# wondmgezahu/RAMP

Measured on AMD Instinct MI355X. Metric: sampled trajectories/sec (H=48, T=25), higher is better.
Workload: dtype f32-emulated (2 x fp16 planes per operand, fp32 accumulate)

## Files before the change

ramp_amd/csrc/args_token.h:

```cpp
#pragma once
#include "core.h"

namespace ramp {

struct FfxArgs {
  int M = 0;
  const float* X = nullptr;
  const float* Z1 = nullptr;
  float* Y = nullptr;
  float* stash = nullptr;
  const float* ln_g = nullptr; const float* ln_b = nullptr;
  const unsigned short* Wstream = nullptr;
  const float* b1 = nullptr;
  const float* b2 = nullptr;
  const float* amax_in1 = nullptr; float* amax_out1 = nullptr; float wsi1 = 1.f; int site1 = 0;
  const float* amax_in2 = nullptr; float* amax_out2 = nullptr; float wsi2 = 1.f; int site2 = 0;
  int* range_flag = nullptr;
  unsigned long long* stamps = nullptr;
  int ablate = 0;
  int tok0 = 0, slot0 = 0, half_mode = 0;
};
int launch_ffx(const FfxArgs& f, bool bwd, hipStream_t s);
int ffx_pack_second(const float* W, int rows, int cols, int mode, float scale, float* tmp, unsigned short* out, hipStream_t s);
int ffx_build_stream(const unsigned short* p1, const unsigned short* p2, unsigned short* out, bool bwd, hipStream_t s);
int init_ffx_attributes();
int launch_ffx16(const FfxArgs& f, bool bwd, hipStream_t s);
int ffx16_pack(const float* W, int rows, int cols, int perm, float scale, float* tmp, unsigned short* out, hipStream_t s);
int ffx16_build_stream(const unsigned short* p1, const unsigned short* p2, unsigned short* out, bool bwd, hipStream_t s);
int init_ffx16_attributes();

struct TklArgs {
  int M = 0, N = 0;
  const float* X = nullptr;
  float* Y = nullptr; int ldy = 0;
  const unsigned short* W = nullptr;
  const float* bias = nullptr;
  const float* resid = nullptr; int ldr = 0;
  const float* rowbias = nullptr; const int* rowvar = nullptr; int row0 = 0, rb_stride = 0, L = 1, n_var = 0;
  const float* ln_g = nullptr; const float* ln_b = nullptr;
  const float* amax_in = nullptr; float* amax_out = nullptr; float wsi = 1.f; int site = 0;
  int* range_flag = nullptr;
  int ablate = 0;
};
// ... 18 lines not shown
```

ramp_amd/csrc/engine.hip:

```cpp
#include "engine_util.h"

#include <algorithm>
#include <array>
#include <cmath>
#include <cstring>
#include <map>
#include <memory>
#include <mutex>
#include <string>
#include <unordered_map>
#include <vector>

namespace ramp {

static thread_local std::string g_err;
void set_last_error(const std::string& msg) { g_err = msg; }
int device_cu_count() {
  static int cached[64] = {0};
  int dev = 0;
  if (hipGetDevice(&dev) != hipSuccess || dev < 0 || dev >= 64) return 256;
  if (!cached[dev]) {
    hipDeviceProp_t p;
    cached[dev] = hipGetDeviceProperties(&p, dev) == hipSuccess && p.multiProcessorCount > 0 ? p.multiProcessorCount : 256;
  }
// ... 22 lines not shown
  float *w1_f = nullptr, *w1_b = nullptr, *b1 = nullptr, *w2_f = nullptr, *w2_b = nullptr, *b2 = nullptr;
  float *w1_pk = nullptr, *b1_pk = nullptr;
  float *ln1_g = nullptr, *ln1_b = nullptr, *ln3_g = nullptr, *ln3_b = nullptr;
  const float *wv2 = nullptr, *wo2 = nullptr, *bo2 = nullptr;
  float *a_qkv = nullptr, *a_z1 = nullptr, *a_ag = nullptr, *a_z2 = nullptr;
  unsigned short *ffx_f = nullptr, *ffx_b = nullptr; float ffx_wsi_w1 = 1.f, ffx_wsi_w2 = 1.f;
  unsigned short *ffx16_f = nullptr, *ffx16_b = nullptr;
  unsigned short* ato_w = nullptr; float ato_wsi = 1.f;
  unsigned short* abl_w = nullptr;
};
struct ST {
  std::string name;
  int C = 0, L = 0, blk0 = 0;
  float *gn_g = nullptr, *gn_b = nullptr, *wpi_f = nullptr, *wpi_b = nullptr, *bpi = nullptr;
  float *wpo_f = nullptr, *wpo_b = nullptr, *bpo = nullptr;
  STBlock blk[2];
  float *a_gst = nullptr, *a_z0 = nullptr, *a_y = nullptr;
};
struct Resample {
  std::string name;
  float *w_f = nullptr, *w_b = nullptr, *bias = nullptr;
  int C = 0, Lin = 0, Lout = 0, taps = 0;
  float* a_y = nullptr;
};

}

using namespace ramp;

#ifndef RAMP_DEFAULT_GEMM_MODE
// ... 32 lines not shown
  bool c_cal_valid = false; std::string c_cal_key; unsigned long long* c_cal_rec = nullptr;
  std::map<std::string, float*> c_cal_saved;
  std::vector<float*> c_cal_free;
  float *r_noise = nullptr, *r_hist = nullptr, *r_xclean = nullptr, *r_best = nullptr, *r_plen = nullptr, *r_smooth = nullptr,
        *r_cost = nullptr, *r_hard_val = nullptr;
  double *r_static = nullptr, *r_dyn = nullptr;
  int *r_mask = nullptr, *r_en = nullptr, *r_result = nullptr, *r_hard_idx = nullptr;
  ReplanState* r_state = nullptr;
  size_t r_cap_B = 0, r_cap_static = 0, r_cap_dyn = 0, r_cap_cost = 0;
  hipGraphExec_t r_graph[2] = {nullptr, nullptr}; std::string r_key;
  bool r_calibrated = false;
  float* scene_ws = nullptr; size_t scene_ws_cap = 0;
  int gemm_mode = 0;
  struct X6W { unsigned short* planes; size_t n; int K; unsigned short* packed; unsigned short* packed3; float w_scale_inv; };
  std::map<const float*, X6W> x6;
  int x6_pipe = 1;
  int geglu_group = 64;
  static constexpr int MAX_SITES = 1024, N_OBS_TABLES = 4;
  int phase = 0, site = 0;
  int ff_fused = 150000;
  int three_blocks = 1;
  int mfma16 = 1;
  int ffx_min_rows = 32768;
  int tkl_min_rows = 65536;
  int atk_min_rows = 40000;
  int tkc_gn = 3;
  int tkc_min_rows = 16384;
  int tkw_min_rows = 16384;
  std::map<const float*, unsigned short*> tk16_w;
  struct TkcW { unsigned short* planes; float wsi; };
// ... 146 lines not shown
    CK(get_raw(c, t + ".norm1.weight", {D}, &k.ln1_g)); CK(get_raw(c, t + ".norm1.bias", {D}, &k.ln1_b));
    CK(get_raw(c, t + ".norm3.weight", {D}, &k.ln3_g)); CK(get_raw(c, t + ".norm3.bias", {D}, &k.ln3_b));
    float* tmp;
    CK(get_raw(c, t + ".attn2.to_v.weight", {D, ctx}, &tmp)); k.wv2 = tmp;
    CK(get_raw(c, t + ".attn2.to_out.0.weight", {D, D}, &tmp)); k.wo2 = tmp;
    CK(get_raw(c, t + ".attn2.to_out.0.bias", {D}, &tmp)); k.bo2 = tmp;
    CK(get_raw(c, t + ".attn2.to_q.weight", {D, D}, &tmp));
    CK(get_raw(c, t + ".attn2.to_k.weight", {D, ctx}, &tmp));
    CK(get_raw(c, t + ".norm2.weight", {D}, &tmp)); CK(get_raw(c, t + ".norm2.bias", {D}, &tmp));
    CK(dev_alloc(c, &k.a_qkv, tok * 768)); CK(dev_alloc(c, &k.a_z1, tok * D));
    CK(dev_alloc(c, &k.a_ag, (tok + 127) * 2048)); CK(dev_alloc(c, &k.a_z2, tok * D));
  }
  return 0;
}

struct Run {
  ramp_ctx* c; hipStream_t s; int R; int row0;
  int prep(GemmArgs& b) {
    if (!(c->gemm_mode >= 1 && (b.N >= 128 || (c->x6_pipe && b.N >= 64)))) return 0;
    auto it = c->x6.upper_bound(b.W);
    if (it == c->x6.begin()) return 0;
    --it;
    const auto& e = it->second;
    if (!(b.W >= it->first && b.W < it->first + e.n)) return 0;
    const size_t off = b.W - it->first;
    const bool frag = c->x6_pipe && e.packed && e.K == b.K && off % (32ul * b.K) == 0 && b.N % 32 == 0;
    if (!frag) { b.Wx = e.planes + off; b.wx_plane = (long)e.n; return 0; }
    RAMP_REQUIRE(c->site < ramp_ctx::MAX_SITES, "too many GEMM call sites for the scale table");
    int kind = 1;
    if (c->phase == 2 && e.packed3) {
// ... 64 lines not shown
  int gemm(const GemmArgs& a) {
    if (const ramp_ctx::TkcW* w = tkc_planes(a)) return tkc(a, *w);
    prof_pre(c, s, CAT_GEMM, 2.0 * a.M * a.N * a.K * a.taps, {a.M, a.N, a.K, a.taps});
    GemmArgs b = a;
    b.three_ok = c->three_blocks;
    const int kind = prep(b);
    if (kind < 0) return kind;
    int rc = launch_gemm(b, s);
    prof_post(c, s);
    c->launches++;
    return rc;
  }
  bool use_ffx(const STBlock& k, int M) const {
    return k.ffx_f && c->ffx_min_rows > 0 && M >= c->ffx_min_rows && c->gemm_mode == 2 && c->phase == 2 && c->x6_pipe;
  }
  int ffx(const STBlock& k, bool bwd, const float* X, const float* z1, float* Y, int M) {
    RAMP_REQUIRE(c->site + 2 <= ramp_ctx::MAX_SITES, "too many GEMM call sites for the scale table");
    prof_pre(c, s, CAT_GEMM, 2.0 * M * (2048.0 * 256 + 256.0 * 1024), {M, bwd ? -3 : -2, 256, 2});
    FfxArgs f; f.M = M; f.X = X; f.Z1 = z1; f.Y = Y; f.stash = k.a_ag; f.ln_g = k.ln3_g; f.ln_b = k.ln3_b;
    const bool s16 = c->mfma16 && k.ffx16_f;
    f.Wstream = s16 ? (bwd ? k.ffx16_b : k.ffx16_f) : (bwd ? k.ffx_b : k.ffx_f); f.b1 = k.b1_pk; f.b2 = k.b2; f.range_flag = c->range_flag;
    f.amax_in1 = c->obs_in + c->site; f.amax_out1 = c->obs_out + c->site; f.site1 = c->site;
    f.amax_in2 = c->obs_in + c->site + 1; f.amax_out2 = c->obs_out + c->site + 1; f.site2 = c->site + 1;
    f.wsi1 = bwd ? k.ffx_wsi_w2 : k.ffx_wsi_w1; f.wsi2 = bwd ? k.ffx_wsi_w1 : k.ffx_wsi_w2;
    f.ablate = s16 ? 0 : c->ffx_ablate;
    c->site += 2;
    int rc = s16 ? launch_ffx16(f, bwd, s) : launch_ffx(f, bwd, s);
    prof_post(c, s);
    c->launches++;
    return rc;
  }
  bool has_h3(const float* W, int N, int K) const {
    auto it = c->x6.upper_bound(W);
    if (it == c->x6.begin()) return false;
    --it;
    const auto& e = it->second;
    if (!(W >= it->first && W < it->first + e.n)) return false;
    const size_t off = W - it->first;
    return c->x6_pipe && e.packed && e.packed3 && e.K == K && off % (32ul * K) == 0 && N % 32 == 0;
  }
  bool use_tkl(const GemmArgs& a) const {
// ... 237 lines not shown
        LAUNCH(c, r.s, CAT_ROW, 0, launch_ln_fwd(zin, k.ln1_g, k.ln1_b, c->t_ln, Mb, r.s));
        CK(r.gemm(q));
      }
    }
    const float* rowbias = c->cross_bias + (size_t)(m.blk0 + b) * D; const int rb_stride = c->n_blocks_total * D;
    if (r.use_ato(k, Mb, m.L)) {
      CK(r.ato(k, k.a_qkv, zin, pre ? c->t_ln : k.a_z1, Mb, m.L, pre ? nullptr : rowbias, rb_stride));
    } else {
    LAUNCH(c, r.s, CAT_ATTN, 16.0 * Rb * m.L * m.L * 64, launch_attn_fwd(k.a_qkv, c->t_o, Rb, m.L, r.s));
    GemmArgs a = lin(c->t_o, D, k.wo_f, k.bo, pre ? c->t_ln : k.a_z1, D, Mb, D, D);
    a.resid = zin; a.ldr = D; a.L = m.L;
    if (!pre) { a.rowbias = rowbias; a.rb_stride = rb_stride; a.rowvar = c->row_variant; a.row0 = r.row0; }
    if (r.use_tkl(a) && (!a.rowbias || c->n_variants <= 4)) CK(r.tkl(a, nullptr, nullptr)); else CK(r.gemm(a));
    }
    if (pre) LAUNCH(c, r.s, CAT_ROW, 0, launch_expand_rows(c->t_ln, k.a_z1, R, share, m.L, D, rowbias, rb_stride, c->row_variant, r.row0, r.s));
    if (r.use_ffx(k, M)) {
      CK(r.ffx(k, false, k.a_z1, k.a_z1, k.a_z2, M));
      zin = k.a_z2;
      continue;
    }
    LAUNCH(c, r.s, CAT_ROW, 0, launch_ln_fwd(k.a_z1, k.ln3_g, k.ln3_b, c->t_ln, M, r.s));
    GemmArgs u = lin(c->t_ln, D, k.w1_pk, k.b1_pk, k.a_ag, 2048, M, 2048, D);
    u.epi = EPI_GEGLU_FWD; u.aux_out = c->t_hg; u.ld_aux = 1024;
    u.geglu_group = c->geglu_group;
    GemmArgs f = lin(c->t_hg, 1024, k.w2_f, k.b2, k.a_z2, D, M, D, 1024);
    f.resid = k.a_z1; f.ldr = D;
    CK(r.ff_forward(u, f));
    zin = k.a_z2;
  }
  GemmArgs o = lin(zin, D, m.wpo_f, m.bpo, m.a_y, m.C, M, m.C, D);
// ... 388 lines not shown
    if (const char* me = getenv("RAMP_MFMA16")) c->mfma16 = atoi(me) != 0;
    const char* ke = getenv("RAMP_TKL");
    if (ke) c->tkl_min_rows = atoi(ke);
    const char* tce = getenv("RAMP_TKC");
    if (tce) c->tkc_min_rows = atoi(tce);
    if (const char* tg = getenv("RAMP_TKC_GN")) c->tkc_gn = atoi(tg) & 3;
    const char* twe = getenv("RAMP_TKW");
    if (twe) c->tkw_min_rows = atoi(twe);
    const char* ate = getenv("RAMP_ATK");
    if (ate) c->atk_min_rows = atoi(ate);
    const char* se = getenv("RAMP_SHARE_PREFIX");
    if (se) c->share_prefix = atoi(se) != 0;
    const char* te = getenv("RAMP_X6_THREE");
    if (te) c->three_blocks = te[0] != '0';
    c->prof_dump = getenv("RAMP_PROFILE_DUMP") != nullptr;
    const char* ae = getenv("RAMP_FFX_ABLATE");
    if (ae) {
      const int av = atoi(ae);
      if (!(av == 0 || av == 16 || av == 32 || av == 48)) {
        delete c;
        RAMP_REQUIRE(false, "RAMP_FFX_ABLATE accepts 0, 16, 32 or 48 (result-preserving variants) on a context; the others change results and exist in ramp_bench_gemm only");
      }
      c->ffx_ablate = av;
    }
    c->tklb_off = getenv("RAMP_TKLB_OFF") != nullptr;
    if (const char* e = getenv("RAMP_ABL")) c->abl_on = atoi(e) != 0;
  }
  *out = c;
  return 0;
}
// ... 194 lines not shown
          const auto& e1 = c->x6.at(k.w1_pk); const auto& e1b = c->x6.at(k.w1_b);
          const auto& e2 = c->x6.at(k.w2_f); const auto& e2b = c->x6.at(k.w2_b);
          RAMP_REQUIRE(e1.packed3 && e2b.packed3 && e1.w_scale_inv == e1b.w_scale_inv && e2.w_scale_inv == e2b.w_scale_inv, "ffx: weight planes missing");
          float *sf, *sb; CK(dev_alloc(c, &sf, 96 * 8192 + 4)); CK(dev_alloc(c, &sb, 96 * 8192 + 4));
          k.ffx_f = reinterpret_cast<unsigned short*>(sf); k.ffx_b = reinterpret_cast<unsigned short*>(sb);
          CK(ffx_pack_second(k.w2_f, 256, 1024, 0, 1.f / e2.w_scale_inv, tmp, p2f, 0));
          CK(ffx_build_stream(e1.packed3, p2f, k.ffx_f, false, 0));
          CK(ffx_pack_second(k.w1_b, 256, 2048, 1, 1.f / e1.w_scale_inv, tmp, p2b, 0));
          CK(ffx_build_stream(e2b.packed3, p2b, k.ffx_b, true, 0));
          k.ffx_wsi_w1 = e1.w_scale_inv; k.ffx_wsi_w2 = e2.w_scale_inv;
          float *sf6, *sb6; CK(dev_alloc(c, &sf6, 96 * 8192 + 4)); CK(dev_alloc(c, &sb6, 96 * 8192 + 4));
          k.ffx16_f = reinterpret_cast<unsigned short*>(sf6); k.ffx16_b = reinterpret_cast<unsigned short*>(sb6);
          CK(ffx16_pack(k.w1_pk, 2048, 256, 0, 1.f / e1.w_scale_inv, tmp, p1x, 0));
          CK(ffx16_pack(k.w2_f, 256, 1024, 1, 1.f / e2.w_scale_inv, tmp, p2f, 0));
          CK(ffx16_build_stream(p1x, p2f, k.ffx16_f, false, 0));
          CK(ffx16_pack(k.w2_b, 1024, 256, 0, 1.f / e2.w_scale_inv, tmp, p1x, 0));
          CK(ffx16_pack(k.w1_b, 256, 2048, 2, 1.f / e1.w_scale_inv, tmp, p2b, 0));
          CK(ffx16_build_stream(p1x, p2b, k.ffx16_b, true, 0));
          for (const auto& wn : {std::make_pair((const float*)k.wqkv_f, 768), std::make_pair((const float*)k.wo_f, 256), std::make_pair((const float*)k.wo_b, 256)}) {
            const auto& ew = c->x6.at(wn.first);
            if (!ew.packed3) continue;
            float* q16; CK(dev_alloc(c, &q16, (size_t)wn.second * 256 + 4));
            CK(ffx16_pack(wn.first, wn.second, 256, 0, 1.f / ew.w_scale_inv, tmp, reinterpret_cast<unsigned short*>(q16), 0));
            c->tk16_w[wn.first] = reinterpret_cast<unsigned short*>(q16);
          }
        }
    }
    if (c->gemm_mode == 2 && c->x6_pipe) {
      for (auto& st : c->sts)
        for (auto& k : st.blk) {
// ... 730 lines not shown
```

ramp_amd/csrc/ffx16.hip:

```cpp
#include "args_token.h"
#include "pack.h"
#include "tokmma.h"
#include "atkmma.h"

#include <algorithm>
#include <type_traits>

namespace ramp {

namespace {

constexpr int F6_SLAB = 32 * 1024;
constexpr int F6_R = 4;
constexpr int F6_B1 = F6_R * F6_SLAB;
constexpr int F6_LN = F6_B1 + 2048 * 4;
constexpr int F6_B2 = F6_LN + 512 * 4;
constexpr size_t F6_LDS = (size_t)F6_R * F6_SLAB + 2048 * 4 + 512 * 4 + 256 * 4;
constexpr int F6_SLABS = 96;
static_assert(F6_LDS <= 160 * 1024, "LDS budget");

enum { Q_P1A = 0, Q_P1B = 1, Q_P2A = 2, Q_P2B = 3 };
template <int V> using QO = std::integral_constant<int, V>;

}

namespace {
__device__ __forceinline__ void split2x(float x0, float x1, float s, unsigned& hi, unsigned& lo) {
  unsigned h, l;
  asm("v_fma_mixlo_f16 %0, %1, %3, 0 op_sel:[0,0,0] op_sel_hi:[0,0,0]\n\t"
      "v_fma_mixhi_f16 %0, %2, %3, 0 op_sel:[0,0,0] op_sel_hi:[0,0,0]"
      : "=&v"(h) : "v"(x0), "v"(x1), "v"(s));
  asm("v_fma_mixlo_f16 %0, %1, %3, -%4 op_sel:[0,0,0] op_sel_hi:[0,0,1]\n\t"
      "v_fma_mixhi_f16 %0, %2, %3, -%4 op_sel:[0,0,1] op_sel_hi:[0,0,1]"
      : "=&v"(l) : "v"(x0), "v"(x1), "v"(s), "v"(h));
  hi = h; lo = l;
}
}

template <bool BWD, int ABL, int NT>
__device__ __forceinline__ void ffx16_body(const FfxArgs& f, int n_mt) {
  static_assert(NT == 1 || NT == 2, "token halves");
  constexpr int NQ = 2 * NT;
  extern __shared__ __attribute__((aligned(16))) char smem[];
  const int tid = threadIdx.x, lane = tid & 63;
  const int wave = __builtin_amdgcn_readfirstlane(tid >> 6);
  const int c = lane & 15, gq = lane >> 4;
  const int n_my = (n_mt - (int)blockIdx.x + (int)gridDim.x - 1) / (int)gridDim.x;

  const float s_1 = scale_of(f.amax_in1), s_2 = scale_of(f.amax_in2);
  const float os1 = f.wsi1 / s_1, os2 = f.wsi2 / s_2;
  float amax1 = 0.f, amax2 = 0.f;
  const unsigned long long t_start = (ABL & 64) ? __builtin_amdgcn_s_memtime() : 0, r_start = (ABL & 64) ? __builtin_amdgcn_s_memrealtime() : 0;

  const char* wsrc = reinterpret_cast<const char*>(f.Wstream) + wave * 8192 + lane * 16;
  int is_q = 0, is_g = 0;
  const char* cur_src = wsrc; unsigned cur_dst = 0;
  auto dma_begin = [&]() __attribute__((always_inline)) {
    cur_src = wsrc + (long)is_q * F6_SLAB;
    cur_dst = (unsigned)(uintptr_t)(smem + (is_g & (F6_R - 1)) * F6_SLAB + wave * 8192);
    is_q = is_q + 1 == F6_SLABS ? 0 : is_q + 1;
    ++is_g;
  };
#define F6_PIECE(C) asm volatile("s_mov_b32 m0, %1\n\ts_nop 0\n\tglobal_load_lds_dwordx4 %0, off offset:%2" \
                                 :: "v"(cur_src + ((C) >> 2) * 4096), "s"(cur_dst + ((C) >> 2) * 4096), "n"(((C) & 3) * 1024) : "memory", "m0")
  auto dma_piece = [&](int cc) __attribute__((always_inline)) {
    switch (cc) { case 0: F6_PIECE(0); break; case 1: F6_PIECE(1); break; case 2: F6_PIECE(2); break; case 3: F6_PIECE(3); break;
                  case 4: F6_PIECE(4); break; case 5: F6_PIECE(5); break; case 6: F6_PIECE(6); break; default: F6_PIECE(7); break; }
  };
  auto issue_slab = [&]() __attribute__((always_inline)) {
    dma_begin();
#pragma unroll
    for (int cc = 0; cc < 8; ++cc) dma_piece(cc);
  };

  u32x4 F[3][4];
// ... 18 lines not shown
  f32x4 st1[BWD ? NQ : 1], st2[BWD ? NQ : 1];
  const f32x4 zero4 = {0.f, 0.f, 0.f, 0.f};

#define F6_MM(ACC, FA, BB, Z) ACC = mm32(FA, BB, (Z) ? zero4 : ACC)

  auto slab = [&](auto kind_c, auto fo_c, int par, auto side, auto vm_c) __attribute__((always_inline)) {
    constexpr int KIND = decltype(kind_c)::value, FO = decltype(fo_c)::value;
    slab_top(vm_c);
    const int slot = g & (F6_R - 1), nslot = (g + 1) & (F6_R - 1);
#pragma unroll
    for (int m = 0; m < 8; ++m) {
      u32x4 (&FB)[4] = F[(m + FO) % 3];
      u32x4 (&FN)[4] = F[(m + 2 + FO) % 3];
      const char* np = rd + (m < 6 ? slot * F6_SLAB + (m + 2) * 4096 : nslot * F6_SLAB + (m - 6) * 4096);
      constexpr bool P1 = KIND == Q_P1A || KIND == Q_P1B;
      const bool Z = P1 && m == 0;
      constexpr int T1 = NT - 1;
      f32x4* X0; f32x4* X1; f32x4* Y0; f32x4* Y1;
      const u32x4 (*BP)[2]; const u32x4 (*BQ)[2];
      if constexpr (!BWD) {
        if constexpr (P1) {
          X0 = &acc1[par][0][KIND]; X1 = &acc1[par][0][2 * T1 + KIND]; Y0 = &acc1[par][1][KIND]; Y1 = &acc1[par][1][2 * T1 + KIND];
          BP = XB[m]; BQ = XB[m];
        } else {
          X0 = &acc2[2 * m][0]; X1 = &acc2[2 * m][T1]; Y0 = &acc2[2 * m + 1][0]; Y1 = &acc2[2 * m + 1][T1];
          BP = HB; BQ = HB;
        }
      } else {
        if constexpr (P1) {
          X0 = &acc1[par][0][0]; X1 = &acc1[par][0][2 * T1]; Y0 = &acc1[par][0][1]; Y1 = &acc1[par][0][2 * T1 + 1];
          BP = XB[m]; BQ = XB[m];
        } else {
          const int nt = 8 * (KIND - Q_P2A) + m;
          X0 = &acc2[nt][0]; X1 = &acc2[nt][T1]; Y0 = X0; Y1 = X1;
          BP = HB; BQ = HB + NT;
// ... 290 lines not shown
      slab(KD{}, QO<0>{}, 0, [&](int m) __attribute__((always_inline)) { E_step(31, 1, 8 + m, 20, 16); }, V8{});
#pragma unroll
      for (int i = 16; i < 20; ++i) E_step(31, 1, i, 20, 16);
      slab(KC{}, QO<2>{}, 0, no_side, V8{}); slab(KD{}, QO<1>{}, 0, no_side, V8{});
    }
    asm volatile("s_nop 15\n\ts_nop 15" ::: "memory");

    int mt_e = mt;
    asm volatile("" : "+s"(mt_e));
    long tok_e[NT];
#pragma unroll
    for (int t = 0; t < NT; ++t) {
      tok_e[t] = (NT == 2 ? (long)mt_e * 128 + wave * 32 : (long)f.tok0 + (long)mt_e * 64 + wave * 16) + 16 * t + c;
      tok_e[t] = tok_e[t] < f.M ? tok_e[t] : f.M - 1;
    }
    if (!BWD) {
      const float* b2s = reinterpret_cast<const float*>(smem + F6_B2) + 4 * gq;
      f32x4 rz[NT][16];
#pragma unroll
      for (int t = 0; t < NT; ++t) {
        const float* zrow = f.Z1 + tok_e[t] * 256 + 4 * gq;
#pragma unroll
        for (int nt = 0; nt < 16; ++nt) rz[t][nt] = *reinterpret_cast<const f32x4*>(zrow + 16 * nt);
      }
#pragma unroll
      for (int t = 0; t < NT; ++t) {
        float* orow = f.Y + tok_e[t] * 256 + 4 * gq;
#pragma unroll
        for (int nt = 0; nt < 16; ++nt) {
          const f32x4 b2 = *reinterpret_cast<const f32x4*>(b2s + 16 * nt);
          const f32x4 v = acc2[nt][t] * os2 + b2 + rz[t][nt];
// ... 52 lines not shown
#undef F6_PIECE
#undef F6_MM
  if ((ABL & 64) && f.stamps && lane == 0) {
    unsigned long long* o = f.stamps + ((long)blockIdx.x * 4 + wave) * 6;
    o[0] = 0; o[1] = 0; o[2] = 0; o[3] = 0;
    o[4] = __builtin_amdgcn_s_memtime() - t_start;
    o[5] = __builtin_amdgcn_s_memrealtime() - r_start;
  }

  asm volatile("s_waitcnt vmcnt(0)" ::: "memory");

#pragma unroll
  for (int o = 32; o > 0; o >>= 1) { amax1 = fmaxf(amax1, __shfl_xor(amax1, o)); amax2 = fmaxf(amax2, __shfl_xor(amax2, o)); }
  record_amax_block(f.amax_out1, amax1, reinterpret_cast<float*>(smem));
  record_amax_block(f.amax_out2, amax2, reinterpret_cast<float*>(smem) + 4);
  if (lane == 0) {
    if (f.range_flag) {
      if (!(amax1 * s_1 < 60000.f) || (amax1 > 0.f && amax1 * s_1 < 0.125f)) atomicMax(f.range_flag, f.site1 + 1);
      if (!(amax2 * s_2 < 60000.f) || (amax2 > 0.f && amax2 * s_2 < 0.125f)) atomicMax(f.range_flag, f.site2 + 1);
    }
  }
}

template <bool BWD, int ABL = 0>
__global__ __launch_bounds__(256) __attribute__((amdgpu_waves_per_eu(1, 1)))
void ffx16_kernel(FfxArgs f, int n_mt) { ffx16_body<BWD, ABL, 2>(f, n_mt); }
template <bool BWD>
__global__ __launch_bounds__(256) __attribute__((amdgpu_waves_per_eu(1, 1)))
void ffx16h_kernel(FfxArgs f, int n_mt) { ffx16_body<BWD, 0, 1>(f, n_mt); }

__global__ void ffx16_gather_kernel(const float* __restrict__ in, float* __restrict__ out, int rows, int cols, int perm) {
  const long total = (long)rows * cols;
  const int oc = cols / 2;
  for (long idx = (long)blockIdx.x * 256 + threadIdx.x; idx < total; idx += (long)gridDim.x * 256) {
    const long orow = idx / oc; const int ocol = (int)(idx - orow * oc);
    const long R = orow >> 5; const int b = (int)(orow >> 4) & 1, cc = (int)orow & 15;
    const int s = ocol >> 4, h = (ocol >> 3) & 1, j = ocol & 7;
    const long srow = 16 * R + cc;
    const int pcol = 32 * s + 16 * h + 8 * b + j;
    const int gq = (pcol >> 3) & 3, jj = pcol & 7;
    int scol = pcol;
    if (perm == 1) scol = (pcol & ~31) + 16 * (jj >> 2) + 4 * gq + (jj & 3);
    else if (perm == 2) { const int u = pcol >> 6, w = (pcol >> 5) & 1; scol = (w ? 1024 : 0) + 32 * u + 16 * (jj >> 2) + 4 * gq + (jj & 3); }
    out[idx] = in[srow * cols + scol];
  }
}
int ffx16_pack(const float* W, int rows, int cols, int perm, float scale, float* tmp, unsigned short* out, hipStream_t s) {
  RAMP_REQUIRE(W && tmp && out && rows % 16 == 0 && cols % 32 == 0 && perm >= 0 && perm <= 2 && (perm != 2 || cols == 2048), "ffx16_pack: bad shape");
  hipLaunchKernelGGL(ffx16_gather_kernel, dim3(1024), dim3(256), 0, s, W, tmp, rows, cols, perm);
  RAMP_HIP_CHECK(hipGetLastError());
  return launch_pack_h3(tmp, out, 2L * rows, cols / 2, scale, s);
}

__global__ void ffx16_build_stream_kernel(const unsigned short* __restrict__ p1, const unsigned short* __restrict__ p2,
                                          unsigned short* __restrict__ out, int bwd) {
  const int q = blockIdx.x;
  int kind, u;
  if (!bwd) {
    if (q < 4) { kind = q & 1; u = q >> 1; }
    else if (q < 94) { const int k = 1 + (q - 4) / 3, j = (q - 4) - 3 * (k - 1); if (j == 0) { kind = Q_P2A; u = k - 1; } else { kind = j - 1; u = k + 1; } }
    else { kind = Q_P2A; u = q - 64; }
  } else {
    if (q < 2) { kind = Q_P1A; u = q; }
    else if (q < 92) { const int k = 1 + (q - 2) / 3, j = (q - 2) - 3 * (k - 1); if (j == 2) { kind = Q_P1A; u = k + 1; } else { kind = Q_P2A + j; u = k - 1; } }
    else { kind = Q_P2A + (q & 1); u = 30 + ((q - 92) >> 1); }
  }
  for (int i = threadIdx.x >> 6; i < 32; i += blockDim.x >> 6) {
    const int m = i >> 2, j = i & 3, lane = threadIdx.x & 63;
    const int pq = j >> 1, plane = j & 1;
    long frag;
    const unsigned short* base;
    if (!bwd) {
      if (kind <= Q_P1B) { base = p1; frag = (long)(4 * u + 2 * pq + kind) * 8 + m; }
      else { base = p2; frag = (long)(2 * m + pq) * 32 + u; }
    } else {
      if (kind == Q_P1A) { base = p1; frag = (long)(2 * u + pq) * 8 + m; }
      else { base = p2; frag = (long)(8 * (kind - Q_P2A) + m) * 64 + 2 * u + pq; }
    }
    reinterpret_cast<u32x4*>(out + ((long)q * 32 + i) * 512)[lane] = reinterpret_cast<const u32x4*>(base + (frag * 2 + plane) * 512)[lane];
  }
}
int ffx16_build_stream(const unsigned short* p1, const unsigned short* p2, unsigned short* out, bool bwd, hipStream_t s) {
  RAMP_REQUIRE(p1 && p2 && out, "ffx16_build_stream: null operand");
  hipLaunchKernelGGL(ffx16_build_stream_kernel, dim3(F6_SLABS), dim3(256), 0, s, p1, p2, out, bwd ? 1 : 0);
  RAMP_HIP_CHECK(hipGetLastError());
  return 0;
}

int launch_ffx16(const FfxArgs& f, bool bwd, hipStream_t s) {
  auto al16 = [](const void* p) { return (reinterpret_cast<uintptr_t>(p) & 15) == 0; };
  RAMP_REQUIRE(f.M > 0 && f.X && f.Y && f.Z1 && f.stash && f.Wstream && f.ln_g && (bwd || (f.ln_b && f.b1 && f.b2)), "ffx16: null operand");
  RAMP_REQUIRE(al16(f.X) && al16(f.Y) && al16(f.Z1) && al16(f.stash) && al16(f.Wstream) && al16(f.ln_g) && al16(f.ln_b) &&
               al16(f.b1) && al16(f.b2), "ffx16: operands must be 16-byte aligned");
  {
    const size_t yb = (size_t)f.M * 256 * 4;
    RAMP_REQUIRE(!ranges_overlap(f.Y, yb, f.X, yb) && !ranges_overlap(f.Y, yb, f.Z1, yb), "ffx16: the output must not overlap X or z1 (no in-place use)");
  }
  const int n_mt = (f.M + 127) / 128, cus = device_cu_count();
  RAMP_REQUIRE(f.half_mode >= 0 && f.half_mode <= 2 && (f.half_mode == 0 || f.ablate == 0), "ffx16: bad tiling mode");
  int n_full = n_mt;
  if (f.half_mode == 2) n_full = 0;
  else if (f.half_mode == 0 && f.ablate == 0) {
    const int r = n_mt % cus;
    if (2 * n_mt <= cus) n_full = 0;
    else if (n_mt > cus && r > 0 && 2 * r <= cus) n_full = n_mt - r;
  }
#define F6_GO(B, A) hipLaunchKernelGGL((ffx16_kernel<B, A>), dim3(std::min(n_full, cus)), dim3(256), F6_LDS, s, f, n_full)
  if (n_full > 0) {
    if (f.ablate == 0) { if (bwd) F6_GO(true, 0); else F6_GO(false, 0); }
    else if (f.ablate == 1) { if (bwd) F6_GO(true, 1); else F6_GO(false, 1); }
    else if (f.ablate == 64) { if (bwd) F6_GO(true, 64); else F6_GO(false, 64); }
    else RAMP_REQUIRE(false, "ffx16: ablation variant not built");
    RAMP_HIP_CHECK(hipGetLastError());
  }
#undef F6_GO
  if (n_full < n_mt) {
    FfxArgs h = f;
    h.tok0 = n_full * 128; h.slot0 = n_full;
    const int n_half = (f.M - h.tok0 + 63) / 64;
    if (bwd) hipLaunchKernelGGL((ffx16h_kernel<true>), dim3(std::min(n_half, cus)), dim3(256), F6_LDS, s, h, n_half);
    else hipLaunchKernelGGL((ffx16h_kernel<false>), dim3(std::min(n_half, cus)), dim3(256), F6_LDS, s, h, n_half);
    RAMP_HIP_CHECK(hipGetLastError());
  }
  return 0;
}

int init_ffx16_attributes() {
#define F6_ATTR(B, A) RAMP_HIP_CHECK(hipFuncSetAttribute(reinterpret_cast<const void*>(&ffx16_kernel<B, A>), hipFuncAttributeMaxDynamicSharedMemorySize, (int)F6_LDS))
  F6_ATTR(false, 0); F6_ATTR(true, 0); F6_ATTR(false, 1); F6_ATTR(true, 1); F6_ATTR(false, 64); F6_ATTR(true, 64);
#undef F6_ATTR
  RAMP_HIP_CHECK(hipFuncSetAttribute(reinterpret_cast<const void*>(&ffx16h_kernel<false>), hipFuncAttributeMaxDynamicSharedMemorySize, (int)F6_LDS));
  RAMP_HIP_CHECK(hipFuncSetAttribute(reinterpret_cast<const void*>(&ffx16h_kernel<true>), hipFuncAttributeMaxDynamicSharedMemorySize, (int)F6_LDS));
  return 0;
}

}
```

Before: 3962.

## Fuse spatial-transformer proj_out GEMM and residual into the second block's FFX kernel

Adds a proj_out tail to the fused feed-forward kernel for the last transformer block. After the FF output plus residual is formed in registers, it is re-split into fp16 planes and multiplied by extra proj_out weight slabs appended to the weight stream, then bias and the block input residual are added and written directly. This removes a separate GEMM launch and the round trip of the 256-wide intermediate through memory. The cost is more register pressure, extra weight slabs in the pipelined stream, and new kernel variants for each channel count. By default it is enabled only for C >= 64 and large M.

```diff
diff --git a/ramp_amd/csrc/args_token.h b/ramp_amd/csrc/args_token.h
--- a/ramp_amd/csrc/args_token.h
+++ b/ramp_amd/csrc/args_token.h
@@ -19,6 +19,9 @@
   unsigned long long* stamps = nullptr;
   int ablate = 0;
   int tok0 = 0, slot0 = 0, half_mode = 0;
+  int C = 0, L = 1, share = 1;
+  const float* xres = nullptr; const float* bpo = nullptr;
+  float wsi3 = 1.f; float* amax_out3 = nullptr;
 };
 int launch_ffx(const FfxArgs& f, bool bwd, hipStream_t s);
 int ffx_pack_second(const float* W, int rows, int cols, int mode, float scale, float* tmp, unsigned short* out, hipStream_t s);
@@ -26,7 +29,8 @@
 int init_ffx_attributes();
 int launch_ffx16(const FfxArgs& f, bool bwd, hipStream_t s);
 int ffx16_pack(const float* W, int rows, int cols, int perm, float scale, float* tmp, unsigned short* out, hipStream_t s);
-int ffx16_build_stream(const unsigned short* p1, const unsigned short* p2, unsigned short* out, bool bwd, hipStream_t s);
+int ffx16_build_stream(const unsigned short* p1, const unsigned short* p2, unsigned short* out, bool bwd, hipStream_t s,
+                       const unsigned short* p3 = nullptr, int C = 0);
 int init_ffx16_attributes();
 
 struct TklArgs {
diff --git a/ramp_amd/csrc/engine.hip b/ramp_amd/csrc/engine.hip
--- a/ramp_amd/csrc/engine.hip
+++ b/ramp_amd/csrc/engine.hip
@@ -60,6 +60,7 @@
   int C = 0, L = 0, blk0 = 0;
   float *gn_g = nullptr, *gn_b = nullptr, *wpi_f = nullptr, *wpi_b = nullptr, *bpi = nullptr;
   float *wpo_f = nullptr, *wpo_b = nullptr, *bpo = nullptr;
+  unsigned short* ffx16_po = nullptr; float po_wsi = 1.f;
   STBlock blk[2];
   float *a_gst = nullptr, *a_z0 = nullptr, *a_y = nullptr;
 };
@@ -122,6 +123,8 @@
   int gemm_mode = 0;
   struct X6W { unsigned short* planes; size_t n; int K; unsigned short* packed; unsigned short* packed3; float w_scale_inv; };
   std::map<const float*, X6W> x6;
+  int ffx_po_rows = 32768;
+  int ffx_po_c32 = 0;
   int x6_pipe = 1;
   int geglu_group = 64;
   static constexpr int MAX_SITES = 1024, N_OBS_TABLES = 4;
@@ -298,6 +301,8 @@
   return 0;
 }
 
+GemmArgs lin(const float* A, int lda, const float* W, const float* bias, float* C, int ldc, int M, int N, int K);
+
 struct Run {
   ramp_ctx* c; hipStream_t s; int R; int row0;
   int prep(GemmArgs& b) {
@@ -392,9 +397,14 @@
   bool use_ffx(const STBlock& k, int M) const {
     return k.ffx_f && c->ffx_min_rows > 0 && M >= c->ffx_min_rows && c->gemm_mode == 2 && c->phase == 2 && c->x6_pipe;
   }
-  int ffx(const STBlock& k, bool bwd, const float* X, const float* z1, float* Y, int M) {
+  struct PoTail { const ST* m; const float* xres; int L; int share; };
+  bool use_po(const ST& m, int M) const {
+    return c->ffx_po_rows > 0 && M >= c->ffx_po_rows && (m.C >= 64 || c->ffx_po_c32) && m.ffx16_po && c->mfma16 && use_ffx(m.blk[1], M);
+  }
+  int ffx(const STBlock& k, bool bwd, const float* X, const float* z1, float* Y, int M, const PoTail* po = nullptr) {
     RAMP_REQUIRE(c->site + 2 <= ramp_ctx::MAX_SITES, "too many GEMM call sites for the scale table");
-    prof_pre(c, s, CAT_GEMM, 2.0 * M * (2048.0 * 256 + 256.0 * 1024), {M, bwd ? -3 : -2, 256, 2});
+    RAMP_REQUIRE(!po || (!bwd && c->mfma16 && k.ffx16_f && po->m->ffx16_po), "ffx: proj_out tail without its stream");
+    prof_pre(c, s, CAT_GEMM, 2.0 * M * (2048.0 * 256 + 256.0 * 1024 + (po ? 256.0 * po->m->C : 0.0)), {M, bwd ? -3 : -2, 256, 2});
     FfxArgs f; f.M = M; f.X = X; f.Z1 = z1; f.Y = Y; f.stash = k.a_ag; f.ln_g = k.ln3_g; f.ln_b = k.ln3_b;
     const bool s16 = c->mfma16 && k.ffx16_f;
     f.Wstream = s16 ? (bwd ? k.ffx16_b : k.ffx16_f) : (bwd ? k.ffx_b : k.ffx_f); f.b1 = k.b1_pk; f.b2 = k.b2; f.range_flag = c->range_flag;
@@ -403,6 +413,14 @@
     f.wsi1 = bwd ? k.ffx_wsi_w2 : k.ffx_wsi_w1; f.wsi2 = bwd ? k.ffx_wsi_w1 : k.ffx_wsi_w2;
     f.ablate = s16 ? 0 : c->ffx_ablate;
     c->site += 2;
+    if (po) {
+      const ST& m = *po->m;
+      GemmArgs o = lin(X, 256, m.wpo_f, m.bpo, Y, m.C, M, m.C, 256);
+      const int kind = prep(o);
+      if (kind < 0) return kind;
+      f.Wstream = m.ffx16_po; f.C = m.C; f.L = po->L; f.share = po->share; f.xres = po->xres; f.bpo = m.bpo; f.wsi3 = m.po_wsi;
+      f.amax_out3 = kind == 2 ? o.a_absmax_out : nullptr;
+    }
     int rc = s16 ? launch_ffx16(f, bwd, s) : launch_ffx(f, bwd, s);
     prof_post(c, s);
     c->launches++;
@@ -670,6 +688,12 @@
     if (r.use_tkl(a) && (!a.rowbias || c->n_variants <= 4)) CK(r.tkl(a, nullptr, nullptr)); else CK(r.gemm(a));
     }
     if (pre) LAUNCH(c, r.s, CAT_ROW, 0, launch_expand_rows(c->t_ln, k.a_z1, R, share, m.L, D, rowbias, rb_stride, c->row_variant, r.row0, r.s));
+    if (b == 1 && r.use_po(m, M)) {
+      Run::PoTail po{&m, x, m.L, share};
+      CK(r.ffx(k, false, k.a_z1, k.a_z1, m.a_y, M, &po));
+      CK(dbg_store(c, "out/" + m.name, m.a_y, (size_t)M * m.C, r.s));
+      return 0;
+    }
     if (r.use_ffx(k, M)) {
       CK(r.ffx(k, false, k.a_z1, k.a_z1, k.a_z2, M));
       zin = k.a_z2;
@@ -1088,6 +1112,8 @@
     const char* te = getenv("RAMP_X6_THREE");
     if (te) c->three_blocks = te[0] != '0';
     c->prof_dump = getenv("RAMP_PROFILE_DUMP") != nullptr;
+    if (const char* po = getenv("RAMP_FFX_PO")) c->ffx_po_rows = atoi(po);
+    if (const char* po = getenv("RAMP_FFX_PO_C32")) c->ffx_po_c32 = atoi(po) != 0;
     const char* ae = getenv("RAMP_FFX_ABLATE");
     if (ae) {
       const int av = atoi(ae);
@@ -1312,6 +1338,14 @@
           CK(ffx16_pack(k.w1_pk, 2048, 256, 0, 1.f / e1.w_scale_inv, tmp, p1x, 0));
           CK(ffx16_pack(k.w2_f, 256, 1024, 1, 1.f / e2.w_scale_inv, tmp, p2f, 0));
           CK(ffx16_build_stream(p1x, p2f, k.ffx16_f, false, 0));
+          if (&k == &st.blk[1]) {
+            const auto& eo = c->x6.at(st.wpo_f);
+            RAMP_REQUIRE(eo.packed3, "ffx: proj_out planes missing");
+            float *so, *po3; CK(dev_alloc(c, &so, (96 + st.C / 32) * 8192 + 4)); CK(dev_alloc(c, &po3, (size_t)st.C * 256 + 4));
+            st.ffx16_po = reinterpret_cast<unsigned short*>(so); st.po_wsi = eo.w_scale_inv;
+            CK(ffx16_pack(st.wpo_f, st.C, 256, 1, 1.f / eo.w_scale_inv, tmp, reinterpret_cast<unsigned short*>(po3), 0));
+            CK(ffx16_build_stream(p1x, p2f, st.ffx16_po, false, 0, reinterpret_cast<unsigned short*>(po3), st.C));
+          }
           CK(ffx16_pack(k.w2_b, 1024, 256, 0, 1.f / e2.w_scale_inv, tmp, p1x, 0));
           CK(ffx16_pack(k.w1_b, 256, 2048, 2, 1.f / e1.w_scale_inv, tmp, p2b, 0));
           CK(ffx16_build_stream(p1x, p2b, k.ffx16_b, true, 0));
diff --git a/ramp_amd/csrc/ffx16.hip b/ramp_amd/csrc/ffx16.hip
--- a/ramp_amd/csrc/ffx16.hip
+++ b/ramp_amd/csrc/ffx16.hip
@@ -20,6 +20,7 @@
 static_assert(F6_LDS <= 160 * 1024, "LDS budget");
 
 enum { Q_P1A = 0, Q_P1B = 1, Q_P2A = 2, Q_P2B = 3 };
+constexpr int Q_PO = 4;
 template <int V> using QO = std::integral_constant<int, V>;
 
 }
@@ -37,9 +38,11 @@
 }
 }
 
-template <bool BWD, int ABL, int NT>
+template <bool BWD, int ABL, int NT, int NPO = 0>
 __device__ __forceinline__ void ffx16_body(const FfxArgs& f, int n_mt) {
   static_assert(NT == 1 || NT == 2, "token halves");
+  static_assert(NPO == 0 || (!BWD && ABL == 0 && (NPO == 1 || NPO == 2 || NPO == 4 || NPO == 8)), "proj_out tail: forward, C = 32 NPO <= 256");
+  constexpr int NSLABS = F6_SLABS + NPO;
   constexpr int NQ = 2 * NT;
   extern __shared__ __attribute__((aligned(16))) char smem[];
   const int tid = threadIdx.x, lane = tid & 63;
@@ -49,7 +52,7 @@
 
   const float s_1 = scale_of(f.amax_in1), s_2 = scale_of(f.amax_in2);
   const float os1 = f.wsi1 / s_1, os2 = f.wsi2 / s_2;
-  float amax1 = 0.f, amax2 = 0.f;
+  float amax1 = 0.f, amax2 = 0.f, amax3 = 0.f, s_3 = 1.f;
   const unsigned long long t_start = (ABL & 64) ? __builtin_amdgcn_s_memtime() : 0, r_start = (ABL & 64) ? __builtin_amdgcn_s_memrealtime() : 0;
 
   const char* wsrc = reinterpret_cast<const char*>(f.Wstream) + wave * 8192 + lane * 16;
@@ -58,7 +61,7 @@
   auto dma_begin = [&]() __attribute__((always_inline)) {
     cur_src = wsrc + (long)is_q * F6_SLAB;
     cur_dst = (unsigned)(uintptr_t)(smem + (is_g & (F6_R - 1)) * F6_SLAB + wave * 8192);
-    is_q = is_q + 1 == F6_SLABS ? 0 : is_q + 1;
+    is_q = is_q + 1 == NSLABS ? 0 : is_q + 1;
     ++is_g;
   };
 #define F6_PIECE(C) asm volatile("s_mov_b32 m0, %1\n\ts_nop 0\n\tglobal_load_lds_dwordx4 %0, off offset:%2" \
@@ -107,11 +110,16 @@
       u32x4 (&FN)[4] = F[(m + 2 + FO) % 3];
       const char* np = rd + (m < 6 ? slot * F6_SLAB + (m + 2) * 4096 : nslot * F6_SLAB + (m - 6) * 4096);
       constexpr bool P1 = KIND == Q_P1A || KIND == Q_P1B;
-      const bool Z = P1 && m == 0;
+      constexpr bool PO = KIND >= Q_PO;
+      const bool Z = (P1 || PO) && m == 0;
       constexpr int T1 = NT - 1;
       f32x4* X0; f32x4* X1; f32x4* Y0; f32x4* Y1;
       const u32x4 (*BP)[2]; const u32x4 (*BQ)[2];
-      if constexpr (!BWD) {
+      if constexpr (PO) {
+        constexpr int S2 = 2 * (PO ? KIND - Q_PO : 0);
+        X0 = &acc2[S2][0]; X1 = &acc2[S2][T1]; Y0 = &acc2[S2 + 1][0]; Y1 = &acc2[S2 + 1][T1];
+        BP = XB[m]; BQ = XB[m];
+      } else if constexpr (!BWD) {
         if constexpr (P1) {
           X0 = &acc1[par][0][KIND]; X1 = &acc1[par][0][2 * T1 + KIND]; Y0 = &acc1[par][1][KIND]; Y1 = &acc1[par][1][2 * T1 + KIND];
           BP = XB[m]; BQ = XB[m];
@@ -432,7 +440,77 @@
       tok_e[t] = (NT == 2 ? (long)mt_e * 128 + wave * 32 : (long)f.tok0 + (long)mt_e * 64 + wave * 16) + 16 * t + c;
       tok_e[t] = tok_e[t] < f.M ? tok_e[t] : f.M - 1;
     }
-    if (!BWD) {
+    if constexpr (NPO > 0) {
+      const float* b2s = reinterpret_cast<const float*>(smem + F6_B2) + 4 * gq;
+      {
+        float mx = 0.f;
+#pragma unroll
+        for (int t = 0; t < NT; ++t) {
+          const float* zrow = f.Z1 + tok_e[t] * 256 + 4 * gq;
+#pragma unroll
+          for (int h = 0; h < 2; ++h) {
+            f32x4 rz[8];
+#pragma unroll
+            for (int j = 0; j < 8; ++j) rz[j] = *reinterpret_cast<const f32x4*>(zrow + 16 * (8 * h + j));
+#pragma unroll
+            for (int j = 0; j < 8; ++j) {
+              const int nt = 8 * h + j;
+              const f32x4 b2 = *reinterpret_cast<const f32x4*>(b2s + 16 * nt);
+              f32x4 z = acc2[nt][t] * os2 + b2 + rz[j];
+              amax_pin(mx, z[0], z[1]); amax_pin(mx, z[2], z[3]);
+              asm volatile("" : "+a"(z));
+              acc2[nt][t] = z;
+            }
+          }
+        }
+#pragma unroll
+        for (int o = 32; o > 0; o >>= 1) mx = fmaxf(mx, __shfl_xor(mx, o));
+        amax3 = fmaxf(amax3, mx);
+        s_3 = scale_from(mx);
+      }
+#pragma unroll
+      for (int t = 0; t < NT; ++t)
+#pragma unroll
+        for (int ks = 0; ks < 8; ++ks) split8(acc2[2 * ks][t] * s_3, acc2[2 * ks + 1][t] * s_3, XB[ks][t][0], XB[ks][t][1]);
+      pin_acc();
+      slab(std::integral_constant<int, Q_PO + 0>{}, QO<0>{}, 0, no_side, V8{});
+      if constexpr (NPO >= 2) slab(std::integral_constant<int, Q_PO + 1>{}, QO<2>{}, 0, no_side, V8{});
+      if constexpr (NPO >= 4) {
+        slab(std::integral_constant<int, Q_PO + 2>{}, QO<1>{}, 0, no_side, V8{});
+        slab(std::integral_constant<int, Q_PO + 3>{}, QO<0>{}, 0, no_side, V8{});
+      }
+      if constexpr (NPO >= 8) {
+        slab(std::integral_constant<int, Q_PO + 4>{}, QO<2>{}, 0, no_side, V8{});
+        slab(std::integral_constant<int, Q_PO + 5>{}, QO<1>{}, 0, no_side, V8{});
+        slab(std::integral_constant<int, Q_PO + 6>{}, QO<0>{}, 0, no_side, V8{});
+        slab(std::integral_constant<int, Q_PO + 7>{}, QO<2>{}, 0, no_side, V8{});
+      }
+      constexpr int FN = (2 * NPO) % 3;
+      if constexpr (FN == 1) {
+#pragma unroll
+        for (int i = 0; i < 4; ++i) { F[0][i] = F[1][i]; F[1][i] = F[2][i]; }
+      } else if constexpr (FN == 2) {
+#pragma unroll
+        for (int i = 0; i < 4; ++i) { const u32x4 t0 = F[0][i]; F[0][i] = F[2][i]; F[1][i] = t0; }
+      }
+      asm volatile("s_nop 15\n\ts_nop 15" ::: "memory");
+      const float os3 = f.wsi3 / s_3;
+#pragma unroll
+      for (int t = 0; t < NT; ++t) {
+        const int tk = (int)tok_e[t], r = tk / f.L, xr = (r / f.share) * f.L + (tk - r * f.L);
+        const float* xrow = f.xres + (long)xr * (NPO * 32) + 4 * gq;
+        const float* brow = f.bpo + 4 * gq;
+        float* orow = f.Y + (long)tk * (NPO * 32) + 4 * gq;
+        f32x4 rx[2 * NPO];
+#pragma unroll
+        for (int nt = 0; nt < 2 * NPO; ++nt) rx[nt] = *reinterpret_cast<const f32x4*>(xrow + 16 * nt);
+#pragma unroll
+        for (int nt = 0; nt < 2 * NPO; ++nt) {
+          const f32x4 b = *reinterpret_cast<const f32x4*>(brow + 16 * nt);
+          *reinterpret_cast<f32x4*>(orow + 16 * nt) = acc2[nt][t] * os3 + b + rx[nt];
+        }
+      }
+    } else if (!BWD) {
       const float* b2s = reinterpret_cast<const float*>(smem + F6_B2) + 4 * gq;
       f32x4 rz[NT][16];
 #pragma unroll
@@ -515,6 +593,7 @@
   for (int o = 32; o > 0; o >>= 1) { amax1 = fmaxf(amax1, __shfl_xor(amax1, o)); amax2 = fmaxf(amax2, __shfl_xor(amax2, o)); }
   record_amax_block(f.amax_out1, amax1, reinterpret_cast<float*>(smem));
   record_amax_block(f.amax_out2, amax2, reinterpret_cast<float*>(smem) + 4);
+  if constexpr (NPO > 0) record_amax_block(f.amax_out3, amax3, reinterpret_cast<float*>(smem) + 8);
   if (lane == 0) {
     if (f.range_flag) {
       if (!(amax1 * s_1 < 60000.f) || (amax1 > 0.f && amax1 * s_1 < 0.125f)) atomicMax(f.range_flag, f.site1 + 1);
@@ -529,6 +608,12 @@
 template <bool BWD>
 __global__ __launch_bounds__(256) __attribute__((amdgpu_waves_per_eu(1, 1)))
 void ffx16h_kernel(FfxArgs f, int n_mt) { ffx16_body<BWD, 0, 1>(f, n_mt); }
+template <int NPO>
+__global__ __launch_bounds__(256) __attribute__((amdgpu_waves_per_eu(1, 1)))
+void ffx16po_kernel(FfxArgs f, int n_mt) { ffx16_body<false, 0, 2, NPO>(f, n_mt); }
+template <int NPO>
+__global__ __launch_bounds__(256) __attribute__((amdgpu_waves_per_eu(1, 1)))
+void ffx16poh_kernel(FfxArgs f, int n_mt) { ffx16_body<false, 0, 1, NPO>(f, n_mt); }
 
 __global__ void ffx16_gather_kernel(const float* __restrict__ in, float* __restrict__ out, int rows, int cols, int perm) {
   const long total = (long)rows * cols;
@@ -554,10 +639,11 @@
 }
 
 __global__ void ffx16_build_stream_kernel(const unsigned short* __restrict__ p1, const unsigned short* __restrict__ p2,
-                                          unsigned short* __restrict__ out, int bwd) {
+                                          unsigned short* __restrict__ out, int bwd, const unsigned short* __restrict__ p3) {
   const int q = blockIdx.x;
   int kind, u;
-  if (!bwd) {
+  if (q >= F6_SLABS) { kind = Q_PO; u = q - F6_SLABS; }
+  else if (!bwd) {
     if (q < 4) { kind = q & 1; u = q >> 1; }
     else if (q < 94) { const int k = 1 + (q - 4) / 3, j = (q - 4) - 3 * (k - 1); if (j == 0) { kind = Q_P2A; u = k - 1; } else { kind = j - 1; u = k + 1; } }
     else { kind = Q_P2A; u = q - 64; }
@@ -571,7 +657,8 @@
     const int pq = j >> 1, plane = j & 1;
     long frag;
     const unsigned short* base;
-    if (!bwd) {
+    if (kind == Q_PO) { base = p3; frag = (long)(2 * u + pq) * 8 + m; }
+    else if (!bwd) {
       if (kind <= Q_P1B) { base = p1; frag = (long)(4 * u + 2 * pq + kind) * 8 + m; }
       else { base = p2; frag = (long)(2 * m + pq) * 32 + u; }
     } else {
@@ -581,9 +668,11 @@
     reinterpret_cast<u32x4*>(out + ((long)q * 32 + i) * 512)[lane] = reinterpret_cast<const u32x4*>(base + (frag * 2 + plane) * 512)[lane];
   }
 }
-int ffx16_build_stream(const unsigned short* p1, const unsigned short* p2, unsigned short* out, bool bwd, hipStream_t s) {
+int ffx16_build_stream(const unsigned short* p1, const unsigned short* p2, unsigned short* out, bool bwd, hipStream_t s,
+                       const unsigned short* p3, int C) {
   RAMP_REQUIRE(p1 && p2 && out, "ffx16_build_stream: null operand");
-  hipLaunchKernelGGL(ffx16_build_stream_kernel, dim3(F6_SLABS), dim3(256), 0, s, p1, p2, out, bwd ? 1 : 0);
+  RAMP_REQUIRE(C == 0 || (p3 && !bwd && (C == 32 || C == 64 || C == 128 || C == 256)), "ffx16_build_stream: bad proj_out tail");
+  hipLaunchKernelGGL(ffx16_build_stream_kernel, dim3(F6_SLABS + C / 32), dim3(256), 0, s, p1, p2, out, bwd ? 1 : 0, p3);
   RAMP_HIP_CHECK(hipGetLastError());
   return 0;
 }
@@ -593,9 +682,13 @@
   RAMP_REQUIRE(f.M > 0 && f.X && f.Y && f.Z1 && f.stash && f.Wstream && f.ln_g && (bwd || (f.ln_b && f.b1 && f.b2)), "ffx16: null operand");
   RAMP_REQUIRE(al16(f.X) && al16(f.Y) && al16(f.Z1) && al16(f.stash) && al16(f.Wstream) && al16(f.ln_g) && al16(f.ln_b) &&
                al16(f.b1) && al16(f.b2), "ffx16: operands must be 16-byte aligned");
+  const bool po = f.C != 0;
+  RAMP_REQUIRE(!po || (!bwd && f.ablate == 0 && (f.C == 32 || f.C == 64 || f.C == 128 || f.C == 256) && f.xres && f.bpo && al16(f.xres) && al16(f.bpo) &&
+                       f.L >= 1 && f.share >= 1 && f.M % (f.L * f.share) == 0), "ffx16: bad proj_out tail");
   {
-    const size_t yb = (size_t)f.M * 256 * 4;
-    RAMP_REQUIRE(!ranges_overlap(f.Y, yb, f.X, yb) && !ranges_overlap(f.Y, yb, f.Z1, yb), "ffx16: the output must not overlap X or z1 (no in-place use)");
+    const size_t xb = (size_t)f.M * 256 * 4, yb = (size_t)f.M * (po ? f.C : 256) * 4;
+    RAMP_REQUIRE(!ranges_overlap(f.Y, yb, f.X, xb) && !ranges_overlap(f.Y, yb, f.Z1, xb), "ffx16: the output must not overlap X or z1 (no in-place use)");
+    RAMP_REQUIRE(!po || !ranges_overlap(f.Y, yb, f.xres, (size_t)(f.M / f.share) * f.C * 4), "ffx16: the output must not overlap the residual");
   }
   const int n_mt = (f.M + 127) / 128, cus = device_cu_count();
   RAMP_REQUIRE(f.half_mode >= 0 && f.half_mode <= 2 && (f.half_mode == 0 || f.ablate == 0), "ffx16: bad tiling mode");
@@ -607,6 +700,21 @@
     else if (n_mt > cus && r > 0 && 2 * r <= cus) n_full = n_mt - r;
   }
 #define F6_GO(B, A) hipLaunchKernelGGL((ffx16_kernel<B, A>), dim3(std::min(n_full, cus)), dim3(256), F6_LDS, s, f, n_full)
+#define F6_PO(K, N, P) hipLaunchKernelGGL((K<P>), dim3(std::min(N, cus)), dim3(256), F6_LDS, s, h, N)
+#define F6_POS(K, N) do { if (f.C == 32) F6_PO(K, N, 1); else if (f.C == 64) F6_PO(K, N, 2); else if (f.C == 128) F6_PO(K, N, 4); else F6_PO(K, N, 8); } while (0)
+  if (po) {
+    FfxArgs h = f;
+    if (n_full > 0) { F6_POS(ffx16po_kernel, n_full); RAMP_HIP_CHECK(hipGetLastError()); }
+    if (n_full < n_mt) {
+      h.tok0 = n_full * 128; h.slot0 = n_full;
+      const int n_half = (f.M - h.tok0 + 63) / 64;
+      F6_POS(ffx16poh_kernel, n_half);
+      RAMP_HIP_CHECK(hipGetLastError());
+    }
+    return 0;
+  }
+#undef F6_POS
+#undef F6_PO
   if (n_full > 0) {
     if (f.ablate == 0) { if (bwd) F6_GO(true, 0); else F6_GO(false, 0); }
     else if (f.ablate == 1) { if (bwd) F6_GO(true, 1); else F6_GO(false, 1); }
@@ -632,6 +740,10 @@
 #undef F6_ATTR
   RAMP_HIP_CHECK(hipFuncSetAttribute(reinterpret_cast<const void*>(&ffx16h_kernel<false>), hipFuncAttributeMaxDynamicSharedMemorySize, (int)F6_LDS));
   RAMP_HIP_CHECK(hipFuncSetAttribute(reinterpret_cast<const void*>(&ffx16h_kernel<true>), hipFuncAttributeMaxDynamicSharedMemorySize, (int)F6_LDS));
+#define F6_ATTR(K) RAMP_HIP_CHECK(hipFuncSetAttribute(reinterpret_cast<const void*>(&K), hipFuncAttributeMaxDynamicSharedMemorySize, (int)F6_LDS))
+  F6_ATTR(ffx16po_kernel<1>); F6_ATTR(ffx16po_kernel<2>); F6_ATTR(ffx16po_kernel<4>); F6_ATTR(ffx16po_kernel<8>);
+  F6_ATTR(ffx16poh_kernel<1>); F6_ATTR(ffx16poh_kernel<2>); F6_ATTR(ffx16poh_kernel<4>); F6_ATTR(ffx16poh_kernel<8>);
+#undef F6_ATTR
   return 0;
 }
 
```

Result: no change. 3976 (median of 6 runs) (+0.4%).
